# ChazzyGordon/LR2PPO

Hardware: AMD Instinct MI355X
Metric: ppo_steps_per_sec (higher is better)
Workload: dtype f32 (GEMMs: split-bf16 x3 on MFMA, fp32 accumulate); 1 GPU; BASELINE metric 'PPO steps/sec (ViT-B+RoBERTa-base, batch 32)': frames uint8 [32,16,3,224,224] + token ids [32,2,196] -> ViT-B/16 + RoBERTa-base (random weights, inference) -> text_emb [32,2,196,768], img_emb [32,16,768] -> LR2PPO stage-3 rollout + update (actor 519M + critic 526M + reward 526M params); batch_per_gpu=32, tags=2, global_batch=32, parallelism=dp1

## Files before the change

### include/lr2ppo_hip.h

```cpp
#ifndef LR2PPO_HIP_H
#define LR2PPO_HIP_H
#include <stdint.h>

#ifdef __cplusplus
extern "C" {
#endif

#define LR2_ERR_ARG (-1)
#define LR2_ERR_SHAPE (-2)
#define LR2_ERR_LAUNCH (-3)

#define LR2_ABI_VERSION 27
int lr2_abi_version(void);
int lr2_device_info(char* name, int len);

typedef struct lr2_epilogue {
  const void* bias;
  const void* resid;
  const void* aux_z;
  void* out;
  void* out_z;
  void* out_hi;
  uint64_t out_lo_off;
  int32_t ld_planes;
  int32_t ld_resid, ld_aux, ld_out, ld_z;
  int32_t act;
  int32_t accumulate;
  float alpha;
  float drop_p;
  uint32_t drop_site;
  uint32_t _pad;
  uint64_t drop_seed;
  void* adam_p;
  void* adam_m;
  void* adam_v;
  double adam_lr, adam_beta1, adam_beta2, adam_eps, adam_weight_decay;
  void* colsum;
  void* colsum_ws;
  const void* drop_seed_dev;
  const void* adam_lr_dev;
} lr2_epilogue;

int lr2_gemm(const void* A, const void* B, int M, int N, int K, int lda, int ldb, int trans_a, int trans_b,
             uint64_t a_bytes, uint64_t b_bytes, int a_planes, uint64_t a_lo_off, int b_planes, uint64_t b_lo_off,
             const lr2_epilogue* epi, void* splitk_ws, int splits, int block_m, int passes, void* stream);

int lr2_gemm_row_split_plan(int M, int N, int K, int* rows_256, int* tail_block_m);
int lr2_gemm_launch_counts(uint64_t counts[3]);
int lr2_gemm256_tile_rows(int M, int N, int* rows);

int lr2_gather_rows(const void* src, const int64_t* index, void* dst, int B, int t_in, int t_out, uint64_t row_elems,
                    uint64_t src_bstride, uint64_t src_tstride, void* stream);
int lr2_gather_rows_bwd(const void* ddst, const int64_t* index, void* dsrc, int B, int t_in, int t_out,
                        uint64_t row_elems, void* stream);
int lr2_copy_rows(const void* src, void* dst, int dst_planes, uint64_t dst_lo_off, int rows, int D, int group,
                  uint64_t dst_gstride, uint64_t dst_off, void* stream);
int lr2_split_planes(const void* src, void* dst_hi, uint64_t lo_off, uint64_t n, void* stream);
int lr2_split_planes_t(const void* src, void* dst_hi, uint64_t lo_off, int R, int C, void* stream);
int lr2_dropout_planes(const void* src, void* dst_hi, uint64_t lo_off, uint64_t n, float drop_p, uint64_t drop_seed,
                       uint32_t drop_site, void* stream);
typedef struct lr2_split_chunk {
  const void* src;
  void* dst_hi;
  uint64_t lo_off;
  uint64_t count;
} lr2_split_chunk;
int lr2_split_planes_multi(const lr2_split_chunk* table_dev, int n_chunks, void* stream);

int lr2_layernorm_fwd(const void* x, const void* gamma, const void* beta, void* out, void* out_hi, uint64_t out_lo_off,
                      void* mean, void* rstd, int rows, int D, float eps, int mode, int group, uint64_t group_stride,
                      void* stream);

int lr2_layernorm_bwd(const void* dy, int group, uint64_t group_stride, const void* x, const void* gamma, const void* mean,
                      const void* rstd, const void* resid_grad, void* dx, void* dxm_hi, uint64_t dxm_lo_off, float drop_p,
                      uint64_t drop_seed, uint32_t drop_site, const void* drop_seed_dev, void* partials, int nblocks, int rows, int D,
                      int mode, float eps, void* stream);
int lr2_colsum_partials_finish(const void* partials, int nblocks, int cols, int ld, void* out, int accumulate,
                               void* stream);
int lr2_colsum(const void* x, int is_planes, uint64_t lo_off, int rows, int cols, int ld, void* partials, int nblocks,
               void* out, void* stream);

int lr2_xattn_fwd(const void* Q, const void* K, const void* V, void* O, int o_planes, uint64_t o_lo_off, int batch,
                  int heads, int Lq, int Lk, int head_dim, float post_scale, void* stream);
int lr2_xattn_bwd(const void* Q, const void* K, const void* V, const void* dO, void* dQ, void* dK, void* dV,
                  int planes, uint64_t q_lo_off, uint64_t kv_lo_off, int batch, int heads, int Lq, int Lk, int head_dim,
                  float post_scale, void* stream);
int lr2_xattn_fwd_wide(const void* Q, const void* K, const void* V, void* O, int o_planes, uint64_t o_lo_off, int batch,
                       int heads, int Lq, int Lk, int head_dim, float post_scale, void* stream);
int lr2_xattn_bwd_wide(const void* Q, const void* K, const void* V, const void* dO, void* dQ, void* dK, void* dV,
                       int planes, uint64_t q_lo_off, uint64_t kv_lo_off, int batch, int heads, int Lq, int Lk, int head_dim,
                       float post_scale, void* stream);
int lr2_xattn_wide_launch_counts(uint64_t counts[2]);

int lr2_self_attn_fwd(const void* q_hi, const void* k_hi, const void* v_hi, uint64_t lo_off, int ld, const int64_t* seg,
                      void* o, void* o_hi, uint64_t o_lo_off, int ld_o, void* lse, float drop_p, uint64_t drop_seed,
                      uint32_t drop_site, int batch, int heads, int L, int head_dim, float scale, void* stream);

int lr2_first_token_attn(const void* q, int ld_q, const void* k_hi, const void* v_hi, uint64_t lo_off, int ld,
                         const int64_t* seg, void* o, int ld_o, int batch, int heads, int L, int head_dim, float scale,
                         void* stream);

int lr2_self_attn_bwd(const void* q_hi, const void* k_hi, const void* v_hi, uint64_t lo_off, int ld, const void* do_hi,
                      uint64_t do_lo_off, int ld_do, const int64_t* seg, void* dq_hi, void* dk_hi, void* dv_hi,
                      uint64_t d_lo_off, int ld_d, const void* o_hi, uint64_t o_lo_off, int ld_o, void* lse_ws, void* dsum_ws,
                      float drop_p, uint64_t drop_seed, uint32_t drop_site, int batch, int heads, int L, int head_dim, float scale,
                      void* stream);
int lr2_self_attn_plan(int batch, int heads, int L, int ld, int ld_do, int* fwd_persistent, int* bwd_persistent);

int lr2_head_fwd(const void* x, const void* w, const void* b, void* y, int rows, int D, int row_step, int row_off,
                 void* stream);
int lr2_head_bwd(const void* x, const void* w, const void* dy, void* dx, void* dw, void* db, int rows, int D,
                 int row_step, int row_off, int total_rows, void* stream);

int lr2_add_period_rows(const void* x, const void* table, void* out, int rows, int D, int period, void* stream);
int lr2_period_rows_grad(const void* dy, void* dtable, int rows, int D, int period, void* stream);

int lr2_ppo_loss(const void* scores, const void* old_scores, const void* rewards, const void* old_value,
                 const void* value, const int64_t* next_state, int ns_len, int rank_len, int B, int T, float kl_w,
                 float ent_w, float value_clip, float margin, float adv_eps, void* scalars, void* per_item,
                 void* dscores, void* dvalue, void* stats_out, const void* global_stats, int world, void* stream);

int lr2_cls_head_fwd(const void* x, const void* w, const void* b, void* y, int rows, int D, int C, void* stream);
int lr2_cls_head_bwd(const void* x, const void* w, const void* dy, void* dx, void* dw, void* db, int rows, int D, int C,
                     void* stream);
int lr2_cls_scores(const void* logits, void* probs, void* scores, int rows, int C, int use_softmax, void* stream);
int lr2_cls_scores_bwd(const void* probs, const void* scores, const void* dscores, void* dlogits, int rows, int C, void* stream);
int lr2_nll_loss(const void* logits, const int64_t* tgts, int rows, int C, void* loss, void* dlogits, void* stream);

int lr2_smooth_l1(const void* pred, const void* target, int n, float beta, void* loss, void* dpred, void* stream);

int lr2_pair_hinge(const void* scores, int bs, float margin, void* loss_acc, void* dscores, void* stream);

// ... 100 lines not shown
```

### lr2ppo_amd/_native.py

```python
from __future__ import annotations

import ctypes as C
import os
import subprocess
import threading

_HERE = os.path.dirname(os.path.abspath(__file__))
CSRC = os.path.join(_HERE, "csrc")
INCLUDE = os.path.join(os.path.dirname(_HERE), "include")
LIB_PATH = os.path.join(CSRC, "liblr2ppo_hip.so")
SOURCES = ["gemm.hip", "gemm256.hip", "gemm256_mx.hip", "gemm256_b1.hip", "gemm256_f16.hip", "gemm256_tn_b1.hip", "norm.hip", "attn.hip", "attn_wide.hip", "selfattn_fwd.hip", "selfattn_bwd.hip", "first_token_attn.hip", "selfattn_mx.hip", "selfattn_mx_blocked.hip","selfattn_b1_train.hip", "selfattn_b1_blocked.hip", "misc.hip", "fp8.hip", "fp8_train.hip"]
HEADERS = [os.path.join(CSRC, "common.h"), os.path.join(CSRC, "gemm_common.h"), os.path.join(CSRC, "gemm256_ring.h"), os.path.join(CSRC, "fp8_common.h"), os.path.join(CSRC, "selfattn_common.h"), os.path.join(CSRC, "selfattn_b1.h"), os.path.join(INCLUDE, "lr2ppo_hip.h")]
EXTRA_FLAGS = {"attn_wide.hip": ["-fno-slp-vectorize"]}

ABI_VERSION = 27

_lock = threading.Lock()
_lib = None
_lib_override = None


def use_library(path: str):
    global _lib_override
    if _lib is not None:
        raise RuntimeError("lr2ppo_amd: the kernel library is already loaded")
    _lib_override = path


def _stale() -> bool:
    if not os.path.exists(LIB_PATH):
        return True
    t = os.path.getmtime(LIB_PATH)
    deps = [os.path.join(CSRC, s) for s in SOURCES] + HEADERS
    return any(os.path.getmtime(d) > t for d in deps if os.path.exists(d))


def build(force: bool = False, verbose: bool = False) -> str:
    if not force and not _stale():
        return LIB_PATH
    hipcc = os.environ.get("HIPCC", "hipcc")
    objs = []
    procs = []
    for s in SOURCES:
        obj = os.path.join(CSRC, s.replace(".hip", ".o"))
        cmd = [hipcc, "--offload-arch=gfx950", "-O3", "-std=c++17", "-fPIC", *EXTRA_FLAGS.get(s, []), "-I", INCLUDE, "-I", CSRC, "-c",
               os.path.join(CSRC, s), "-o", obj]
        if verbose:
            print(" ".join(cmd))
        procs.append((s, subprocess.Popen(cmd, stdout=subprocess.PIPE, stderr=subprocess.STDOUT)))
        objs.append(obj)
    for s, p in procs:
        out, _ = p.communicate()
        if p.returncode != 0:
            raise RuntimeError(f"hipcc failed on {s}:\n{out.decode(errors='replace')}")
    cmd = [hipcc, "--offload-arch=gfx950", "-shared", "-fPIC", "-o", LIB_PATH] + objs
    r = subprocess.run(cmd, stdout=subprocess.PIPE, stderr=subprocess.STDOUT)
    if r.returncode != 0:
        raise RuntimeError("link failed:\n" + r.stdout.decode(errors="replace"))
    return LIB_PATH


class Epilogue(C.Structure):
    _fields_ = [("bias", C.c_void_p), ("resid", C.c_void_p), ("aux_z", C.c_void_p), ("out", C.c_void_p),
                ("out_z", C.c_void_p), ("out_hi", C.c_void_p), ("out_lo_off", C.c_uint64), ("ld_planes", C.c_int32),
                ("ld_resid", C.c_int32), ("ld_aux", C.c_int32), ("ld_out", C.c_int32),
                ("ld_z", C.c_int32), ("act", C.c_int32), ("accumulate", C.c_int32), ("alpha", C.c_float),
                ("drop_p", C.c_float), ("drop_site", C.c_uint32), ("_pad", C.c_uint32), ("drop_seed", C.c_uint64),
                ("adam_p", C.c_void_p), ("adam_m", C.c_void_p), ("adam_v", C.c_void_p), ("adam_lr", C.c_double),
                ("adam_beta1", C.c_double), ("adam_beta2", C.c_double), ("adam_eps", C.c_double),
                ("adam_weight_decay", C.c_double), ("colsum", C.c_void_p), ("colsum_ws", C.c_void_p), ("drop_seed_dev", C.c_void_p), ("adam_lr_dev", C.c_void_p)]


class SplitChunk(C.Structure):
    _fields_ = [("src", C.c_void_p), ("dst_hi", C.c_void_p), ("lo_off", C.c_uint64), ("count", C.c_uint64)]


class AdamChunk(C.Structure):
    _fields_ = [("p", C.c_void_p), ("g", C.c_void_p), ("m", C.c_void_p), ("v", C.c_void_p), ("count", C.c_uint64),
                ("weight_decay", C.c_float), ("_pad", C.c_float)]


_P, _I, _F, _U64, _U32 = C.c_void_p, C.c_int, C.c_float, C.c_uint64, C.c_uint32

SIGNATURES = {
    "lr2_abi_version": [],
    "lr2_device_info": [C.c_char_p, _I],
    "lr2_gemm": [_P, _P, _I, _I, _I, _I, _I, _I, _I, _U64, _U64, _I, _U64, _I, _U64, C.POINTER(Epilogue), _P, _I, _I, _I, _P],
    "lr2_gemm_row_split_plan": [_I, _I, _I, C.POINTER(C.c_int), C.POINTER(C.c_int)],
    "lr2_gemm_launch_counts": [C.POINTER(C.c_uint64)],
    "lr2_gemm256_tile_rows": [_I, _I, C.POINTER(C.c_int)],
    "lr2_gather_rows": [_P, _P, _P, _I, _I, _I, _U64, _U64, _U64, _P],
    "lr2_gather_rows_bwd": [_P, _P, _P, _I, _I, _I, _U64, _P],
    "lr2_copy_rows": [_P, _P, _I, _U64, _I, _I, _I, _U64, _U64, _P],
    "lr2_split_planes": [_P, _P, _U64, _U64, _P],
    "lr2_dropout_planes": [_P, _P, _U64, _U64, _F, _U64, _U32, _P],
    "lr2_dropout_apply": [_P, _P, _U64, _F, _U64, _U32, _P],
    "lr2_text_embed_bwd": [_P, _P, _P, _P, _P, _P, _P, _P, _I, _I, C.c_int64, _I, _P],
    "lr2_split_planes_t": [_P, _P, _U64, _I, _I, _P],
    "lr2_split_planes_multi": [_P, _I, _P],
    "lr2_layernorm_fwd": [_P, _P, _P, _P, _P, _U64, _P, _P, _I, _I, _F, _I, _I, _U64, _P],
    "lr2_layernorm_bwd": [_P, _I, _U64, _P, _P, _P, _P, _P, _P, _P, _U64, _F, _U64, _U32, _P, _P, _I, _I, _I, _I, _F, _P],
    "lr2_colsum_partials_finish": [_P, _I, _I, _I, _P, _I, _P],
    "lr2_colsum": [_P, _I, _U64, _I, _I, _I, _P, _I, _P, _P],
    "lr2_xattn_fwd": [_P, _P, _P, _P, _I, _U64, _I, _I, _I, _I, _I, _F, _P],
    "lr2_xattn_bwd": [_P, _P, _P, _P, _P, _P, _P, _I, _U64, _U64, _I, _I, _I, _I, _I, _F, _P],
    "lr2_xattn_fwd_wide": [_P, _P, _P, _P, _I, _U64, _I, _I, _I, _I, _I, _F, _P],
    "lr2_xattn_bwd_wide": [_P, _P, _P, _P, _P, _P, _P, _I, _U64, _U64, _I, _I, _I, _I, _I, _F, _P],
    "lr2_xattn_wide_launch_counts": [C.POINTER(C.c_uint64)],
    "lr2_self_attn_fwd": [_P, _P, _P, _U64, _I, _P, _P, _P, _U64, _I, _P, _F, _U64, _U32, _I, _I, _I, _I, _F, _P],
    "lr2_first_token_attn": [_P, _I, _P, _P, _U64, _I, _P, _P, _I, _I, _I, _I, _I, _F, _P],
    "lr2_self_attn_bwd": [_P, _P, _P, _U64, _I, _P, _U64, _I, _P, _P, _P, _P, _U64, _I, _P, _U64, _I, _P, _P, _F, _U64, _U32, _I,
                          _I, _I, _I, _F, _P],
    "lr2_self_attn_plan": [_I, _I, _I, _I, _I, C.POINTER(C.c_int), C.POINTER(C.c_int)],
    "lr2_head_fwd": [_P, _P, _P, _P, _I, _I, _I, _I, _P],
    "lr2_head_bwd": [_P, _P, _P, _P, _P, _P, _I, _I, _I, _I, _I, _P],
    "lr2_add_period_rows": [_P, _P, _P, _I, _I, _I, _P],
    "lr2_period_rows_grad": [_P, _P, _I, _I, _I, _P],
    "lr2_ppo_loss": [_P, _P, _P, _P, _P, _P, _I, _I, _I, _I, _F, _F, _F, _F, _F, _P, _P, _P, _P, _P, _P, _I, _P],
    "lr2_smooth_l1": [_P, _P, _I, _F, _P, _P, _P],
    "lr2_cls_head_fwd": [_P, _P, _P, _P, _I, _I, _I, _P],
    "lr2_cls_head_bwd": [_P, _P, _P, _P, _P, _P, _I, _I, _I, _P],
    "lr2_cls_scores": [_P, _P, _P, _I, _I, _I, _P],
    "lr2_cls_scores_bwd": [_P, _P, _P, _P, _I, _I, _P],
    "lr2_nll_loss": [_P, _P, _I, _I, _P, _P, _P],
    "lr2_pair_hinge": [_P, _I, _F, _P, _P, _P],
    "lr2_adamw_multi": [_P, _I, C.c_double, C.c_double, C.c_double, C.c_double, _P, _P],
    "lr2_step_scalars_store": [_P, _U64, _P, _I, _P],
    "lr2_quant_mxfp8": [_P, _I, _P, _P, _I, _I, _P],
    "lr2_layernorm_fwd_mxfp8": [_P, _P, _P, _P, _P, _P, _I, _I, _F, _I, _P],
    "lr2_gemm_mxfp8": [_P, _P, _P, _P, _P, _I, _P, _P, _I, _I, _P, _P, _P, _U64, _I, _I, _I, _I, _P],
    "lr2_quant_mxfp8_t": [_P, _I, _U64, _I, _P, _I, _I, _P, _P, _P, _P, _P, _P, _I, _I, _I, _P],
    "lr2_gemm_mxfp8_wgrad": [_P, _P, _P, _P, _P, _I, _I, _P, _I, _I, _I, _I, _P],
    "lr2_dropout_residual": [_P, _P, _P, _U64, _F, _U64, _U32, _P],
    "lr2_self_attn_fwd_bf16": [_P, _P, _P, _I, _P, _P, _P, _P, _P, _I, _I, _I, _I, _I, _F, _P],
    "lr2_self_attn_fwd_bf16_plan": [_I, _I, _I, _I, C.POINTER(C.c_int)],
    "lr2_gemm_bf16": [_P, _P, _I, _I, _I, _I, _I, _U64, _U64, C.POINTER(Epilogue), _I, _P],
    "lr2_gemm_bf16_launch_counts": [C.POINTER(C.c_uint64)],
    "lr2_gemm_bf16_train": [_P, _P, _I, _I, _I, _I, _I, _I, _I, _U64, _U64, C.POINTER(Epilogue), _P, _I, _I, _P],
    "lr2_gemm_bf16_train_launch_counts": [C.POINTER(C.c_uint64)],
    "lr2_self_attn_fwd_bf16_train": [_P, _P, _P, _I, _P, _P, _I, _P, _F, _U64, _U32, _I, _I, _I, _I, _F, _P],
    "lr2_self_attn_bwd_bf16": [_P, _P, _P, _I, _P, _I, _P, _P, _P, _P, _I, _P, _P, _F, _U64, _U32, _I, _I, _I, _I, _F, _P],
    "lr2_self_attn_bf16_train_launch_counts": [C.POINTER(C.c_uint64)],
    "lr2_self_attn_fwd_bf16_train_blocked": [_P, _P, _P, _I, _P, _P, _I, _P, _F, _U64, _U32, _I, _I, _I, _I, _F, _P],
    "lr2_self_attn_bwd_bf16_blocked": [_P, _P, _P, _I, _P, _I, _P, _P, _P, _P, _I, _P, _P, _F, _U64, _U32, _I, _I, _I, _I, _F, _P],
    "lr2_self_attn_bf16_blocked_plan": [_I, C.POINTER(C.c_int), C.POINTER(C.c_int), C.POINTER(C.c_int)],
    "lr2_self_attn_bf16_blocked_launch_counts": [C.POINTER(C.c_uint64)],
    "lr2_self_attn_fwd_bf16_blocked": [_P, _P, _P, _I, _P, _P, _P, _P, _P, _I, _I, _I, _I, _I, _F, _P],
    "lr2_self_attn_fwd_bf16_blocked_launch_count": [C.POINTER(C.c_uint64)],
    "lr2_gemm_f16": [_P, _P, _I, _I, _I, _I, _I, _U64, _U64, C.POINTER(Epilogue), _P],
    "lr2_gemm_f16_launch_count": [C.POINTER(C.c_uint64)],
    "lr2_gemm_f16_tiled": [_P, _P, _I, _I, _I, _I, _I, _U64, _U64, C.POINTER(Epilogue), _I, _P],
    "lr2_gemm_f16_launch_counts": [C.POINTER(C.c_uint64)],
    "lr2_layernorm_fwd_f16": [_P, _P, _P, _P, _P, _P, _P, _I, _I, _F, _I, _I, _U64, _P],
    "lr2_round_f16": [_P, _P, _U64, _P],
    "lr2_self_attn_fwd_f16": [_P, _P, _P, _I, _P, _P, _P, _I, _I, _I, _I, _I, _F, _P],
    "lr2_self_attn_fwd_f16_launch_count": [C.POINTER(C.c_uint64)],
    "lr2_self_attn_fwd_f16_blocked": [_P, _P, _P, _I, _P, _P, _P, _I, _I, _I, _I, _I, _F, _P],
    "lr2_self_attn_fwd_f16_blocked_launch_count": [C.POINTER(C.c_uint64)],
    "lr2_text_embed": [_P, _P, _P, _P, _P, _P, _I, _I, _I, C.c_int64, _I, _P, _P],
    "lr2_patchify_planes": [_P, _I, _P, _U64, _I, _I, _I, _I, _I, _I, C.POINTER(C.c_float), C.POINTER(C.c_float), _P],
    "lr2_ndcg": [_P, _P, _P, _P, _P, _I, _P, _I, _P],
    "lr2_patchify": [_P, _P, _I, _I, _I, _I, _I, _P],
    "lr2_vit_assemble": [_P, _P, _P, _P, _I, _I, _I, _P],
}


def lib() -> C.CDLL:
    global _lib
    if _lib is not None:
        return _lib
    with _lock:
        if _lib is not None:
            return _lib
# ... 37 lines not shown
```

### lr2ppo_amd/csrc/gemm256.hip

```cpp
#include "gemm256_ring.h"

namespace lr2gemm {
namespace g256 {

using namespace ring256;
constexpr int BM = 256, BN = 256, BK = 32;
constexpr int LDS_BYTES = RING;

struct SplitProducts {
  template <int AH, int BH, int MIH>
  static __device__ __forceinline__ void mfma_section(f32x4_t (&acc)[2 * MIH][4], const bf16x8_t (&ahi)[MIH], const bf16x8_t (&alo)[MIH],
                                                      const bf16x8_t (&bhi)[2], const bf16x8_t (&blo)[2]) {
    __builtin_amdgcn_s_setprio(1);
#pragma unroll
    for (int j = 0; j < 2; ++j)
#pragma unroll
      for (int i = 0; i < MIH; ++i)
        acc[AH * MIH + i][BH * 2 + j] = __builtin_amdgcn_mfma_f32_16x16x32_bf16(alo[i], bhi[j], acc[AH * MIH + i][BH * 2 + j], 0, 0, 0);
#pragma unroll
    for (int j = 0; j < 2; ++j)
#pragma unroll
      for (int i = 0; i < MIH; ++i)
        acc[AH * MIH + i][BH * 2 + j] = __builtin_amdgcn_mfma_f32_16x16x32_bf16(ahi[i], blo[j], acc[AH * MIH + i][BH * 2 + j], 0, 0, 0);
#pragma unroll
    for (int j = 0; j < 2; ++j)
#pragma unroll
      for (int i = 0; i < MIH; ++i)
        acc[AH * MIH + i][BH * 2 + j] = __builtin_amdgcn_mfma_f32_16x16x32_bf16(ahi[i], bhi[j], acc[AH * MIH + i][BH * 2 + j], 0, 0, 0);
    __builtin_amdgcn_s_setprio(0);
    section_barrier();
  }
};

template <int MIH>
__global__ __launch_bounds__(512, 2) void gemm256_nt_kernel(GemmParams g) {
  constexpr int BMT = 64 * MIH, WMT = 32 * MIH;
  extern __shared__ __attribute__((aligned(16))) char smem[];
  const int tid = threadIdx.x;
  const int lane = tid & 63;
  const int wave = __builtin_amdgcn_readfirstlane(tid >> 6);
  const int wr = wave >> 2, wc = wave & 3;

  int tm, tn;
  tile_coords(g.tiles_m, g.tiles_n, blockIdx.x, tm, tn);
  const int m0 = tm * BMT, n0 = tn * BN;

  Ctx<TwoPlanes> c;
  c.nt = g.K / BK;
  c.src.a = uniform_rsrc(g.A, g.a_bytes);
  c.src.a2 = uniform_rsrc((const char*)g.A + g.a_lo_off, g.a_bytes);
  c.src.b = uniform_rsrc(g.B, g.b_bytes);
  c.src.b2 = uniform_rsrc((const char*)g.B + g.b_lo_off, g.b_bytes);
  lane_setup<MIH>(c, smem, m0, n0, wave, lane, (uint64_t)g.lda * 2u, (uint64_t)g.ldb * 2u, g.M, g.N);

  f32x4_t acc[2 * MIH][4];
#pragma unroll
  for (int i = 0; i < 2 * MIH; ++i)
#pragma unroll
    for (int j = 0; j < 4; ++j) acc[i][j] = f32x4_t{0.f, 0.f, 0.f, 0.f};

  prologue<NoExtras>(c, wr);
  for (int t = 0; t < c.nt; t += 2) {
    k_step_bf16<SplitProducts, 0, MIH>(c, t, acc);
    if (t + 1 < c.nt) k_step_bf16<SplitProducts, 1, MIH>(c, t + 1, acc);
  }
  drain(wr);

  float* slab = reinterpret_cast<float*>(smem) + wave * (32 * (64 + 4));
  epilogue_wave<WMT, 64, 2 * MIH, 4, 1>(g, acc, slab, m0 + wr * WMT, n0 + wc * 64, lane, nullptr);
}

}

namespace g256t {

using g256::BK;
using g256::BM;
using g256::BN;
using ring256::OOB;
constexpr int PLANE = 32 * 256;
constexpr int STAGE_STRIDE = 2 * PLANE;
constexpr int HALF_STRIDE = 2 * STAGE_STRIDE;
constexpr int REGION = 2 * HALF_STRIDE;
constexpr int LDS_BYTES = 2 * REGION;

__device__ __forceinline__ int swz_tr16(int k) { return ((((k & 3) | (((k >> 3) & 1) << 2))) << 1) & 15; }

template <int IMM>
__device__ __forceinline__ bf16x8_t lds_read_tr(uint32_t addr) {
  u32x2_t lo, hi;
  asm volatile("ds_read_b64_tr_b16 %0, %1 offset:%2" : "=v"(lo) : "v"(addr), "i"(IMM));
  asm volatile("ds_read_b64_tr_b16 %0, %1 offset:%2" : "=v"(hi) : "v"(addr), "i"(IMM + 4 * 256));
  u32x4_t v = {lo[0], lo[1], hi[0], hi[1]};
  return __builtin_bit_cast(bf16x8_t, v);
}

struct Ctx {
  __amdgpu_buffer_rsrc_t a_hi, a_lo, b_hi, b_lo;
  uint32_t voff_a[2], voff_b[2];
  uint32_t kstep_a, kstep_b;
  uint32_t rd_a[4], rd_b[2];
  char* smem;
  int wave, nt;
};

template <bool IS_A, int HALF>
__device__ __forceinline__ void issue_part(const Ctx& c, int tile, int stage) {
  const uint32_t base = IS_A ? c.voff_a[HALF] : c.voff_b[HALF];
  const uint32_t step = IS_A ? c.kstep_a : c.kstep_b;
  const uint64_t o = (uint64_t)base + (uint64_t)(uint32_t)tile * (uint64_t)step;
  const uint32_t v = (tile < c.nt && base != OOB && o < (uint64_t)OOB) ? (uint32_t)o : OOB;
  char* dst = c.smem + (IS_A ? 0 : REGION) + HALF * HALF_STRIDE + stage * STAGE_STRIDE + c.wave * 1024;
  __builtin_amdgcn_raw_ptr_buffer_load_lds(IS_A ? c.a_hi : c.b_hi, LDS_PTR(dst), 16, v, 0, 0, 0);
  __builtin_amdgcn_raw_ptr_buffer_load_lds(IS_A ? c.a_lo : c.b_lo, LDS_PTR(dst + PLANE), 16, v, 0, 0, 0);
}

template <int HALF, int S>
__device__ __forceinline__ void read_a_half(const Ctx& c, bf16x8_t (&hi)[4], bf16x8_t (&lo)[4]) {
  constexpr int O = HALF * HALF_STRIDE + S * STAGE_STRIDE;
  hi[0] = lds_read_tr<O>(c.rd_a[0]);
  hi[1] = lds_read_tr<O>(c.rd_a[1]);
  hi[2] = lds_read_tr<O>(c.rd_a[2]);
  hi[3] = lds_read_tr<O>(c.rd_a[3]);
  lo[0] = lds_read_tr<O + PLANE>(c.rd_a[0]);
  lo[1] = lds_read_tr<O + PLANE>(c.rd_a[1]);
  lo[2] = lds_read_tr<O + PLANE>(c.rd_a[2]);
  lo[3] = lds_read_tr<O + PLANE>(c.rd_a[3]);
}
template <int HALF, int S>
__device__ __forceinline__ void read_b_half(const Ctx& c, bf16x8_t (&hi)[2], bf16x8_t (&lo)[2]) {
  constexpr int O = HALF * HALF_STRIDE + S * STAGE_STRIDE;
  hi[0] = lds_read_tr<O>(c.rd_b[0]);
  hi[1] = lds_read_tr<O>(c.rd_b[1]);
  lo[0] = lds_read_tr<O + PLANE>(c.rd_b[0]);
  lo[1] = lds_read_tr<O + PLANE>(c.rd_b[1]);
}

__device__ __forceinline__ float frag_sum(const bf16x8_t& f) {
  const u32x4_t w = __builtin_bit_cast(u32x4_t, f);
  float s = 0.f;
#pragma unroll
  for (int d = 0; d < 4; ++d) s += __uint_as_float(w[d] << 16) + __uint_as_float(w[d] & 0xffff0000u);
  return s;
}
template <int AH>
__device__ __forceinline__ void colsum_frags(float (&cs)[2], int wc, const bf16x8_t (&ahi)[4], const bf16x8_t (&alo)[4]) {
  if (wc == 0) cs[AH] += frag_sum(ahi[0]) + frag_sum(alo[0]);
  else if (wc == 1) cs[AH] += frag_sum(ahi[1]) + frag_sum(alo[1]);
  else if (wc == 2) cs[AH] += frag_sum(ahi[2]) + frag_sum(alo[2]);
  else cs[AH] += frag_sum(ahi[3]) + frag_sum(alo[3]);
}

// ... 65 lines not shown
    const int sx = swz_tr16(ka);
    const uint32_t sm = (uint32_t)(uintptr_t)(__attribute__((address_space(3))) char*)smem;
    const uint32_t rowb = (uint32_t)(ka * 256 + 8 * (pp & 1));
#pragma unroll
    for (int i = 0; i < 4; ++i) c.rd_a[i] = sm + rowb + (uint32_t)((((wr * 8 + 2 * i + (pp >> 1)) ^ sx)) * 16);
#pragma unroll
    for (int j = 0; j < 2; ++j) c.rd_b[j] = sm + REGION + rowb + (uint32_t)((((wc * 4 + 2 * j + (pp >> 1)) ^ sx)) * 16);
  }

  f32x4_t acc[8][4];
#pragma unroll
  for (int i = 0; i < 8; ++i)
#pragma unroll
    for (int j = 0; j < 4; ++j) acc[i][j] = f32x4_t{0.f, 0.f, 0.f, 0.f};

  issue_part<true, 0>(c, 0, 0);
  issue_part<false, 1>(c, 0, 0);
  issue_part<true, 1>(c, 0, 0);
  issue_part<false, 0>(c, 0, 0);
  issue_part<true, 0>(c, 1, 1);
  issue_part<false, 1>(c, 1, 1);
  issue_part<true, 1>(c, 1, 1);
  ring256::end_load_section<6>();
  if (wr == 1) {
    __builtin_amdgcn_s_barrier();
    __builtin_amdgcn_sched_barrier(0);
  }
  float cs[2] = {0.f, 0.f};
  const bool cs_on = g.epi.colsum_partial != nullptr;
  int cs_phase = (t0 + g.tiles_n - tn) % g.tiles_n;
  for (int t = 0; t < c.nt; t += 2) {
    k_step<0>(c, t, acc, cs, wc, cs_on && cs_phase == 0);
    cs_phase = cs_phase + 1 == g.tiles_n ? 0 : cs_phase + 1;
    if (t + 1 < c.nt) k_step<1>(c, t + 1, acc, cs, wc, cs_on && cs_phase == 0);
    cs_phase = cs_phase + 1 == g.tiles_n ? 0 : cs_phase + 1;
  }
  if (wr == 0) {
    __builtin_amdgcn_s_barrier();
    __builtin_amdgcn_sched_barrier(0);
  }
  asm volatile("s_waitcnt vmcnt(0)" ::: "memory");
  __builtin_amdgcn_s_barrier();
  __builtin_amdgcn_sched_barrier(0);

  if (cs_on) {
    float* dst = g.epi.colsum_partial + (size_t)(split * g.tiles_n + tn) * (size_t)g.M;
#pragma unroll
    for (int h = 0; h < 2; ++h) {
      float v = cs[h];
      v += __shfl_xor(v, 16, 64);
      v += __shfl_xor(v, 32, 64);
      const int m = m0 + wr * 128 + h * 64 + wc * 16 + (lane & 15);
      if (lane < 16 && m < g.M) dst[m] = v;
    }
  }
  float* slab = reinterpret_cast<float*>(smem) + wave * (32 * (64 + 4));
  float* partial = g.partial ? g.partial + (size_t)split * (size_t)g.M * (size_t)g.N : nullptr;
  epilogue_wave<128, 64, 8, 4, 1>(g, acc, slab, m0 + wr * 128, n0 + wc * 64, lane, partial);
}

}

int launch_gemm256_tn(const GemmParams& p_in, int splits, hipStream_t stream) {
  using namespace g256t;
  GemmParams p = p_in;
  p.tiles_m = (p.M + BM - 1) / BM;
  p.tiles_n = (p.N + BN - 1) / BN;
  p.splits = splits;
  static bool attr_set = false;
  if (!attr_set) {
    if (lr2_allow_dynamic_lds(gemm256_tn_kernel, LDS_BYTES, "gemm256_tn")) return LR2_ERR_LAUNCH;
    attr_set = true;
  }
  LR2_LAUNCH(gemm256_tn_kernel, dim3(p.tiles_m * p.tiles_n * splits), dim3(512), LDS_BYTES, stream, p);
  return lr2_launch_status(__func__);
}

int gemm256_nt_tile_rows(int M, int N) {
  const int tn = (N + g256::BN - 1) / g256::BN;
  const int t256 = ((M + 255) / 256) * tn, t192 = ((M + 191) / 192) * tn;
  return (t256 < 256 && t192 <= 256 && t192 > t256) ? 192 : 256;
}

int launch_gemm256_nt(const GemmParams& p_in, hipStream_t stream) {
  using namespace g256;
  GemmParams p = p_in;
  const int bm = gemm256_nt_tile_rows(p.M, p.N);
  p.tiles_m = (p.M + bm - 1) / bm;
  p.tiles_n = (p.N + BN - 1) / BN;
  static bool attr_set = false;
  if (!attr_set) {
    if (lr2_allow_dynamic_lds(gemm256_nt_kernel<4>, LDS_BYTES, "gemm256")) return LR2_ERR_LAUNCH;
    if (lr2_allow_dynamic_lds(gemm256_nt_kernel<3>, LDS_BYTES, "gemm256(192 rows)")) return LR2_ERR_LAUNCH;
    attr_set = true;
  }
  if (bm == 192) LR2_LAUNCH(gemm256_nt_kernel<3>, dim3(p.tiles_m * p.tiles_n), dim3(512), LDS_BYTES, stream, p);
  else LR2_LAUNCH(gemm256_nt_kernel<4>, dim3(p.tiles_m * p.tiles_n), dim3(512), LDS_BYTES, stream, p);
  return lr2_launch_status(__func__);
}

}
```

### lr2ppo_amd/csrc/gemm256_ring.h

```cpp
#pragma once
#include "gemm_common.h"

namespace lr2gemm {
namespace ring256 {

constexpr int PLANE = 128 * 64;
constexpr int PART = 2 * PLANE;
constexpr int STAGE = 4 * PART;
constexpr int RING = 2 * STAGE;
constexpr int SLOT_A0 = 0, SLOT_B0 = 1, SLOT_B1 = 2, SLOT_A1 = 3;
constexpr uint32_t OOB = 0xFFFFFF00u;

__device__ __forceinline__ int swz(int r) { return (4 - ((r >> 2) & 3)) & 3; }

template <int IMM>
__device__ __forceinline__ u32x4_t lds_read16(uint32_t addr) {
  u32x4_t v;
  asm volatile("ds_read_b128 %0, %1 offset:%2" : "=v"(v) : "v"(addr), "i"(IMM));
  return v;
}

__device__ __forceinline__ void section_barrier() {
  __builtin_amdgcn_sched_barrier(0);
  __builtin_amdgcn_s_barrier();
// ... 69 lines not shown
  const uint32_t v0 = in ? base + (uint32_t)tile * SRC::STEP : OOB;
  const uint32_t v1 = in ? v0 + SRC::SECOND : OOB;
  char* dst = c.smem + stage * STAGE + SLOT * PART + c.wave * 1024;
  dma16(IS_A ? c.src.a : c.src.b, dst, v0);
  dma16(c.src.template second<IS_A>(), dst + PLANE, v1);
}

template <int SLOT, int MIH, class V>
__device__ __forceinline__ void read_a_half(uint32_t base, V (&p0)[MIH], V (&p1)[MIH]) {
  p0[0] = __builtin_bit_cast(V, lds_read16<SLOT * PART + 0 * 1024>(base));
  p0[1] = __builtin_bit_cast(V, lds_read16<SLOT * PART + 1 * 1024>(base));
  p0[2] = __builtin_bit_cast(V, lds_read16<SLOT * PART + 2 * 1024>(base));
  if constexpr (MIH == 4) p0[3] = __builtin_bit_cast(V, lds_read16<SLOT * PART + 3 * 1024>(base));
  p1[0] = __builtin_bit_cast(V, lds_read16<SLOT * PART + PLANE + 0 * 1024>(base));
  p1[1] = __builtin_bit_cast(V, lds_read16<SLOT * PART + PLANE + 1 * 1024>(base));
  p1[2] = __builtin_bit_cast(V, lds_read16<SLOT * PART + PLANE + 2 * 1024>(base));
  if constexpr (MIH == 4) p1[3] = __builtin_bit_cast(V, lds_read16<SLOT * PART + PLANE + 3 * 1024>(base));
}
template <int SLOT, class V>
__device__ __forceinline__ void read_b_half(uint32_t base, V (&p0)[2], V (&p1)[2]) {
  p0[0] = __builtin_bit_cast(V, lds_read16<SLOT * PART + 0 * 1024>(base));
  p0[1] = __builtin_bit_cast(V, lds_read16<SLOT * PART + 1 * 1024>(base));
  p1[0] = __builtin_bit_cast(V, lds_read16<SLOT * PART + PLANE + 0 * 1024>(base));
  p1[1] = __builtin_bit_cast(V, lds_read16<SLOT * PART + PLANE + 1 * 1024>(base));
}

template <class PRODUCTS, int S, int MIH, class CTX>
__device__ __forceinline__ void k_step_bf16(const CTX& c, int t, f32x4_t (&acc)[2 * MIH][4]) {
  bf16x8_t a0[MIH], a1[MIH], b0[2], b1[2];
  issue_part<SLOT_B0, false, 0>(c, t + 1, S ^ 1);
  read_a_half<SLOT_A0, MIH>(c.rd_a[S], a0, a1);
  read_b_half<SLOT_B0>(c.rd_b[S], b0, b1);
  end_load_section<12>();
  PRODUCTS::template mfma_section<0, 0, MIH>(acc, a0, a1, b0, b1);
  issue_part<SLOT_A0, true, 0>(c, t + 2, S);
  read_b_half<SLOT_B1>(c.rd_b[S], b0, b1);
  end_load_section<12>();
  PRODUCTS::template mfma_section<0, 1, MIH>(acc, a0, a1, b0, b1);
  issue_part<SLOT_B1, false, 1>(c, t + 2, S);
  read_a_half<SLOT_A1, MIH>(c.rd_a[S], a0, a1);
  end_load_section<12>();
  PRODUCTS::template mfma_section<1, 1, MIH>(acc, a0, a1, b0, b1);
  issue_part<SLOT_A1, true, 1>(c, t + 2, S);
  read_b_half<SLOT_B0>(c.rd_b[S], b0, b1);
  end_load_section<6>();
  PRODUCTS::template mfma_section<1, 0, MIH>(acc, a0, a1, b0, b1);
}

struct NoExtras {
  static constexpr int FIRST_WAIT = 6;
  template <class CTX> static __device__ __forceinline__ void begin(const CTX&) {}
  template <class CTX> static __device__ __forceinline__ void after_a1(const CTX&, int) {}
};

template <class EXTRAS, class CTX>
__device__ __forceinline__ void prologue(const CTX& c, int wr) {
  EXTRAS::begin(c);
  issue_part<SLOT_A0, true, 0>(c, 0, 0);
  issue_part<SLOT_B1, false, 1>(c, 0, 0);
  issue_part<SLOT_A1, true, 1>(c, 0, 0);
  EXTRAS::after_a1(c, 0);
  issue_part<SLOT_B0, false, 0>(c, 0, 0);
  issue_part<SLOT_A0, true, 0>(c, 1, 1);
  issue_part<SLOT_B1, false, 1>(c, 1, 1);
  issue_part<SLOT_A1, true, 1>(c, 1, 1);
  EXTRAS::after_a1(c, 1);
  end_load_section<EXTRAS::FIRST_WAIT>();
  if (wr == 1) {
    __builtin_amdgcn_s_barrier();
    __builtin_amdgcn_sched_barrier(0);
  }
}

__device__ __forceinline__ void drain(int wr) {
  if (wr == 0) {
    __builtin_amdgcn_s_barrier();
    __builtin_amdgcn_sched_barrier(0);
  }
  asm volatile("s_waitcnt vmcnt(0)" ::: "memory");
  __builtin_amdgcn_s_barrier();
  __builtin_amdgcn_sched_barrier(0);
}

}
}
```

### lr2ppo_amd/ops.py

```python
from __future__ import annotations

import contextlib
import ctypes as C
import functools
import os
from typing import Optional

import torch

from . import _native as _nat

_PASSES = 3


def set_gemm_passes(p: int):
    global _PASSES
    if p not in (1, 3):
        raise ValueError("passes must be 1 or 3")
    _PASSES = p


def get_gemm_passes() -> int:
    return _PASSES

# ... 395 lines not shown
    e.bias, e.resid, e.out = _ptr(bias), _ptr(resid), _ptr(out)
    e.ld_resid, e.ld_out = _ld(resid, N), (N if ld_out is None else ld_out)
    if out_plane is not None:
        e.out_hi, e.out_lo_off, e.ld_planes = _plane_ptr(out_plane, M * N, "gemm_bf16: out_plane"), 0, N
    elif out_planes is not None:
        if out_planes.rows != M or planes_col < 0 or planes_col % 4 or planes_col + N > out_planes.cols:
            raise ValueError("gemm_bf16: out_planes must be [M, >= planes_col + N], planes_col a multiple of 4")
        e.out_hi, e.out_lo_off, e.ld_planes = out_planes.data_ptr() + 2 * planes_col, out_planes.lo_off, out_planes.cols
    e.act, e.alpha = act, alpha
    if block_m is None:
        block_m = 256 if use_gemm256_b1(M, N, K) else _bf16_fallback_block_m(M, N)
    with _Timed(f"gemm_bf16_M{M}_N{N}_K{K}", 2.0 * M * N * K, 2.0 * (M * K + N * K) + (4.0 if out is not None else 2.0) * M * N):
        rc = _nat.lib().lr2_gemm_bf16(a_ptr, b_ptr, M, N, K, lda, ldb, a.numel() * 2, b.numel() * 2, C.byref(e), block_m, _stream())
    if rc:
        _nat.check(rc, f"lr2_gemm_bf16(M={M},N={N},K={K},block_m={block_m})")
    return out if out is not None else (out_plane if out_plane is not None else out_planes)


def gemm_bf16_launch_counts():
    c = (C.c_uint64 * 2)()
    _nat.check(_nat.lib().lr2_gemm_bf16_launch_counts(c), "lr2_gemm_bf16_launch_counts")
    return int(c[0]), int(c[1])


def gemm_f16(a: torch.Tensor, b: torch.Tensor, out: Optional[torch.Tensor], M: int, N: int, K: int, *,
             lda: Optional[int] = None, ldb: Optional[int] = None, ld_out: Optional[int] = None, bias: Optional[torch.Tensor] = None,
             act: int = 0, resid: Optional[torch.Tensor] = None, alpha: float = 1.0, out_plane: Optional[torch.Tensor] = None,
             out_planes: Optional[Planes] = None, planes_col: int = 0, block_m: Optional[int] = None):
    _chk_f32(out, bias, resid)
    lda = K if lda is None else lda
    ldb = K if ldb is None else ldb
    a_ptr = _plane_ptr(a, (M - 1) * lda + K, "gemm_f16: a")
    b_ptr = _plane_ptr(b, (N - 1) * ldb + K, "gemm_f16: b")
    if out_plane is not None and out_planes is not None:
        raise ValueError("gemm_f16: out_plane excludes out_planes")
    e = _nat.Epilogue()
    e.bias, e.resid, e.out = _ptr(bias), _ptr(resid), _ptr(out)
    e.ld_resid, e.ld_out = _ld(resid, N), (N if ld_out is None else ld_out)
    if out_plane is not None:
        e.out_hi, e.out_lo_off, e.ld_planes = _plane_ptr(out_plane, M * N, "gemm_f16: out_plane"), 0, N
    elif out_planes is not None:
        if out_planes.rows != M or planes_col < 0 or planes_col % 4 or planes_col + N > out_planes.cols:
            raise ValueError("gemm_f16: out_planes must be [M, >= planes_col + N], planes_col a multiple of 4")
        e.out_hi, e.out_lo_off, e.ld_planes = out_planes.data_ptr() + 2 * planes_col, out_planes.lo_off, out_planes.cols
    e.act, e.alpha = act, alpha
    with _Timed(f"gemm_f16_M{M}_N{N}_K{K}", 2.0 * M * N * K, 2.0 * (M * K + N * K) + (4.0 if out is not None else 2.0) * M * N):
        if block_m is None:
            rc = _nat.lib().lr2_gemm_f16(a_ptr, b_ptr, M, N, K, lda, ldb, a.numel() * 2, b.numel() * 2, C.byref(e), _stream())
        else:
            if block_m not in (256, 128, 64):
                raise ValueError("gemm_f16: block_m is None, 256, 128 or 64")
            rc = _nat.lib().lr2_gemm_f16_tiled(a_ptr, b_ptr, M, N, K, lda, ldb, a.numel() * 2, b.numel() * 2, C.byref(e), block_m,
                                               _stream())
    if rc:
        _nat.check(rc, f"lr2_gemm_f16(M={M},N={N},K={K},block_m={block_m})")
    return out if out is not None else (out_plane if out_plane is not None else out_planes)


def gemm_f16_launch_count() -> int:
    c = C.c_uint64(0)
    _nat.check(_nat.lib().lr2_gemm_f16_launch_count(C.byref(c)), "lr2_gemm_f16_launch_count")
    return int(c.value)


def gemm_f16_launch_counts():
    c = (C.c_uint64 * 2)()
    _nat.check(_nat.lib().lr2_gemm_f16_launch_counts(c), "lr2_gemm_f16_launch_counts")
    return int(c[0]), int(c[1])


_F16_FORCE_256 = False


@contextlib.contextmanager
def f16_force_256():
    global _F16_FORCE_256
    prev, _F16_FORCE_256 = _F16_FORCE_256, True
    try:
        yield
    finally:
        _F16_FORCE_256 = prev


def f16_schedule_block_m(M: int, N: int, K: int) -> Optional[int]:
    return None if _F16_FORCE_256 else f16_block_m(M, N, K)


@functools.lru_cache(maxsize=4096)
def f16_block_m(M: int, N: int, K: int) -> int:
    if K % 64:
        return 64
    tiles = ((M + 255) // 256) * ((N + 255) // 256)
    return 256 if tiles >= 128 else 64


def layernorm_fwd_f16(x, gamma, beta, rows, D, eps, mode, *, group=0, group_stride=0, out=None, mean=None, rstd=None,
                      out_plane: Optional[torch.Tensor] = None):
    _chk_f32(x, gamma, beta, out, mean, rstd)
    if out is None and out_plane is None:
        raise ValueError("layernorm_fwd_f16: out and / or out_plane")
    hp = _plane_ptr(out_plane, rows * D, "layernorm_fwd_f16: out_plane") if out_plane is not None else None
    with _Timed(f"lnfwd_f16_R{rows}_D{D}", 0.0, (6.0 if out is None else 10.0 if out_plane is not None else 8.0) * rows * D):
        rc = _nat.lib().lr2_layernorm_fwd_f16(x.data_ptr(), gamma.data_ptr(), beta.data_ptr(), _ptr(out), hp, _ptr(mean), _ptr(rstd),
                                              rows, D, eps, mode, group, group_stride, _stream())
    _nat.check(rc, "lr2_layernorm_fwd_f16")
    return out if out is not None else out_plane


def round_f16(src: torch.Tensor, dst: torch.Tensor) -> torch.Tensor:
    _chk_f32(src)
    n = src.numel()
    with _Timed(f"round_f16_{n}", 0.0, 6.0 * n):
        rc = _nat.lib().lr2_round_f16(src.data_ptr(), _plane_ptr(dst, n, "round_f16: dst"), n, _stream())
    _nat.check(rc, "lr2_round_f16")
    return dst


def self_attn_fwd_f16(qkv: torch.Tensor, seg, *, batch, heads, L, head_dim, scale, out: Optional[torch.Tensor] = None,
                      out_plane: Optional[torch.Tensor] = None):
    E = heads * head_dim
    if qkv.element_size() != 2 or not qkv.is_cuda or qkv.numel() < batch * L * 3 * E:
        raise TypeError("self_attn_fwd_f16: qkv is a 2-byte HIP tensor [batch * L, 3 * heads * head_dim]")
    if seg.dtype != torch.int64:
        raise TypeError("seg must be int64")
    _chk_f32(out)
    if out is None and out_plane is None:
        raise ValueError("self_attn_fwd_f16: out and / or out_plane")
    ob = _plane_ptr(out_plane, batch * L * E, "self_attn_fwd_f16: out_plane") if out_plane is not None else None
    base = qkv.data_ptr()
    with _Timed(f"selfattn_f16_B{batch}_H{heads}_L{L}", 4.0 * batch * heads * L * L * head_dim, 7.0 * batch * L * E):
        _nat.check(_nat.lib().lr2_self_attn_fwd_f16(base, base + 2 * E, base + 4 * E, 3 * E, seg.data_ptr(), _ptr(out), ob, E, batch,
                                                    heads, L, head_dim, scale, _stream()), "lr2_self_attn_fwd_f16")
    return out if out is not None else out_plane


def self_attn_fwd_f16_launch_count() -> int:
    c = C.c_uint64(0)
    _nat.check(_nat.lib().lr2_self_attn_fwd_f16_launch_count(C.byref(c)), "lr2_self_attn_fwd_f16_launch_count")
    return int(c.value)


def self_attn_fwd_f16_blocked(qkv: torch.Tensor, seg, *, batch, heads, L, head_dim, scale, out: Optional[torch.Tensor] = None,
                              out_plane: Optional[torch.Tensor] = None):
    E = heads * head_dim
    if qkv.element_size() != 2 or not qkv.is_cuda or qkv.numel() < batch * L * 3 * E:
        raise TypeError("self_attn_fwd_f16_blocked: qkv is a 2-byte HIP tensor [batch * L, 3 * heads * head_dim]")
    if seg.dtype != torch.int64:
        raise TypeError("seg must be int64")
    _chk_f32(out)
    if out is None and out_plane is None:
        raise ValueError("self_attn_fwd_f16_blocked: out and / or out_plane")
    ob = _plane_ptr(out_plane, batch * L * E, "self_attn_fwd_f16_blocked: out_plane") if out_plane is not None else None
    base = qkv.data_ptr()
    with _Timed(f"selfattn_f16l_B{batch}_H{heads}_L{L}", 4.0 * batch * heads * L * L * head_dim, 7.0 * batch * L * E):
        _nat.check(_nat.lib().lr2_self_attn_fwd_f16_blocked(base, base + 2 * E, base + 4 * E, 3 * E, seg.data_ptr(), _ptr(out), ob, E,
                                                            batch, heads, L, head_dim, scale, _stream()), "lr2_self_attn_fwd_f16_blocked")
    return out if out is not None else out_plane


def self_attn_fwd_f16_blocked_launch_count() -> int:
    c = C.c_uint64(0)
    _nat.check(_nat.lib().lr2_self_attn_fwd_f16_blocked_launch_count(C.byref(c)), "lr2_self_attn_fwd_f16_blocked_launch_count")
    return int(c.value)


_BF16_TRAIN_FORCE_256 = False
# ... 706 lines not shown
```

Baseline: 14.36 PPO steps/s (1 step = ViT-B/16 over 32 x 16 frames + RoBERTa-base over 32 x 2 tag sequences, frozen, in line -> 1 rollout batch + 1 update minibatch, 32 items x 2 tags per GPU; head_only_steps_per_sec = the same step on pre-extracted features).

## Add persistent 256x256 NT GEMM kernel that prefetches next tile during tail

Adds a persistent variant of the 256-row NT GEMM kernel that launches one workgroup per CU and walks multiple output tiles. The last K-steps of each tile issue loads for the next tile's first stages, so the next tile's prologue overlaps the current epilogue and launch/ramp costs are amortised. By default it is used only for large GEMMs (at least 4x CU-count tiles) whose epilogue loads nothing extra (no residual, accumulate or Adam). It reserves extra LDS for the epilogue slab, which may lower occupancy, and the cross-tile pipeline adds synchronisation complexity.

Result: no change. 14.45 PPO steps/s (1 step = ViT-B/16 over 32 x 16 frames + RoBERTa-base over 32 x 2 tag sequences, frozen, in line -> 1 rollout batch + 1 update minibatch, 32 items x 2 tags per GPU; head_only_steps_per_sec = the same step on pre-extracted features) (median of 6 runs) (+0.6%).

```diff
diff --git a/include/lr2ppo_hip.h b/include/lr2ppo_hip.h
--- a/include/lr2ppo_hip.h
+++ b/include/lr2ppo_hip.h
@@ -48,6 +48,8 @@
 int lr2_gemm_row_split_plan(int M, int N, int K, int* rows_256, int* tail_block_m);
 int lr2_gemm_launch_counts(uint64_t counts[3]);
 int lr2_gemm256_tile_rows(int M, int N, int* rows);
+int lr2_gemm256_persist_plan(int M, int N, int K);
+int lr2_gemm256_persist(int mode, int workgroups);
 
 int lr2_gather_rows(const void* src, const int64_t* index, void* dst, int B, int t_in, int t_out, uint64_t row_elems,
                     uint64_t src_bstride, uint64_t src_tstride, void* stream);
diff --git a/lr2ppo_amd/_native.py b/lr2ppo_amd/_native.py
--- a/lr2ppo_amd/_native.py
+++ b/lr2ppo_amd/_native.py
@@ -89,6 +89,8 @@
     "lr2_gemm_row_split_plan": [_I, _I, _I, C.POINTER(C.c_int), C.POINTER(C.c_int)],
     "lr2_gemm_launch_counts": [C.POINTER(C.c_uint64)],
     "lr2_gemm256_tile_rows": [_I, _I, C.POINTER(C.c_int)],
+    "lr2_gemm256_persist_plan": [_I, _I, _I],
+    "lr2_gemm256_persist": [_I, _I],
     "lr2_gather_rows": [_P, _P, _P, _I, _I, _I, _U64, _U64, _U64, _P],
     "lr2_gather_rows_bwd": [_P, _P, _P, _I, _I, _I, _U64, _P],
     "lr2_copy_rows": [_P, _P, _I, _U64, _I, _I, _I, _U64, _U64, _P],
diff --git a/lr2ppo_amd/csrc/gemm256.hip b/lr2ppo_amd/csrc/gemm256.hip
--- a/lr2ppo_amd/csrc/gemm256.hip
+++ b/lr2ppo_amd/csrc/gemm256.hip
@@ -68,6 +68,85 @@
 
   float* slab = reinterpret_cast<float*>(smem) + wave * (32 * (64 + 4));
   epilogue_wave<WMT, 64, 2 * MIH, 4, 1>(g, acc, slab, m0 + wr * WMT, n0 + wc * 64, lane, nullptr);
+}
+
+template <int FORM>
+__global__ __launch_bounds__(512, 2) void gemm256_nt_persist_kernel(GemmParams g) {
+  constexpr int MIH = 4, BMT = 64 * MIH, WMT = 32 * MIH;
+  extern __shared__ __attribute__((aligned(16))) char smem[];
+  const int total = g.tiles_m * g.tiles_n;
+  int v = blockIdx.x;
+  if (v >= total) return;
+  const int tid = threadIdx.x;
+  const int lane = tid & 63;
+  const int wave = __builtin_amdgcn_readfirstlane(tid >> 6);
+  const int wr = wave >> 2, wc = wave & 3;
+  const uint64_t pitch_a = (uint64_t)g.lda * 2u, pitch_b = (uint64_t)g.ldb * 2u;
+
+  int tm, tn;
+  tile_coords(g.tiles_m, g.tiles_n, v, tm, tn);
+  int m0 = tm * BMT, n0 = tn * BN;
+
+  Ctx<TwoPlanes> c;
+  c.nt = g.K / BK;
+  c.src.a = uniform_rsrc(g.A, g.a_bytes);
+  c.src.a2 = uniform_rsrc((const char*)g.A + g.a_lo_off, g.a_bytes);
+  c.src.b = uniform_rsrc(g.B, g.b_bytes);
+  c.src.b2 = uniform_rsrc((const char*)g.B + g.b_lo_off, g.b_bytes);
+  lane_setup<MIH>(c, smem, m0, n0, wave, lane, pitch_a, pitch_b, g.M, g.N);
+  float* slab = reinterpret_cast<float*>(smem + WALK_KEEP) + wave * (32 * (64 + 4));
+
+  for (bool first = true;; first = false) {
+    const int vn = v + (int)gridDim.x;
+    const bool more = vn < total;
+    int m0n = 0, n0n = 0;
+    if (more) {
+      tile_coords(g.tiles_m, g.tiles_n, vn, tm, tn);
+      m0n = tm * BMT;
+      n0n = tn * BN;
+    }
+    NextTile nx;
+    next_tile_offsets<MIH>(c, nx, more, m0n, n0n, lane, pitch_a, pitch_b, g.M, g.N);
+
+    f32x4_t acc[2 * MIH][4];
+#pragma unroll
+    for (int i = 0; i < 2 * MIH; ++i)
+#pragma unroll
+      for (int j = 0; j < 4; ++j) acc[i][j] = f32x4_t{0.f, 0.f, 0.f, 0.f};
+
+    if (first) prologue<NoExtras>(c, wr);
+    else walk_skew(wr);
+    for (int t = 0; t < c.nt - 2; t += 2) {
+      k_step_bf16_stage0<SplitProducts, MIH>(c, t, acc, !first && t == 0);
+      k_step_bf16<SplitProducts, 1, MIH>(c, t + 1, acc);
+    }
+    k_step_walk<SplitProducts, 0, MIH>(c, nx, acc, !first && c.nt == 2);
+    k_step_walk<SplitProducts, 1, MIH>(c, nx, acc, false);
+    drain(wr);
+
+    GemmParams ge = g;
+    if constexpr (FORM >= 1) {
+      ge.epi.aux_z = nullptr;
+      ge.epi.accumulate = 0;
+      ge.epi.adam_p = nullptr;
+    }
+    if constexpr (FORM == 1) {
+      ge.epi.resid = nullptr;
+      ge.epi.act = g.epi.act & 1u;
+    }
+    epilogue_wave<WMT, 64, 2 * MIH, 4, 1>(ge, acc, slab, m0 + wr * WMT, n0 + wc * 64, lane, nullptr);
+    if (!more) break;
+    walk_release();
+#pragma unroll
+    for (int h = 0; h < 2; ++h) {
+      c.voff_a[h] = nx.voff_a[h];
+      c.voff_b[h] = nx.voff_b[h];
+    }
+    walk_restart(c);
+    m0 = m0n;
+    n0 = n0n;
+    v = vn;
+  }
 }
 
 }
@@ -299,21 +378,71 @@
   return (t256 < 256 && t192 <= 256 && t192 > t256) ? 192 : 256;
 }
 
+static int persist_cus() {
+  static int cached[64] = {0};
+  int dev = 0;
+  if (hipGetDevice(&dev) != hipSuccess || dev < 0 || dev >= 64) {
+    (void)hipGetLastError();
+    return 256;
+  }
+  if (cached[dev] == 0) {
+    int n = 0;
+    if (hipDeviceGetAttribute(&n, hipDeviceAttributeMultiprocessorCount, dev) != hipSuccess || n < 8) n = 256;
+    (void)hipGetLastError();
+    cached[dev] = n & ~7;
+  }
+  return cached[dev];
+}
+
+static int g_persist_mode = 1;
+static int g_persist_wg = 0;
+
+int gemm256_persist_workgroups(int M, int N, int K) {
+  if (g_persist_mode == 0 || M <= 0 || N <= 0 || K <= 0 || (K % 64) != 0) return 0;
+  const int G = g_persist_wg > 0 ? g_persist_wg : persist_cus();
+  if (g_persist_mode == 2) return G;
+  const long long tiles = (long long)((M + 255) / 256) * (long long)((N + g256::BN - 1) / g256::BN);
+  return (gemm256_nt_tile_rows(M, N) == 256 && tiles >= 4ll * G) ? G : 0;
+}
+
+static int persist_form(const GemmParams& p) {
+  const Epilogue& e = p.epi;
+  const bool loads = e.act == 2 || e.resid || e.accumulate;
+  return (!loads && !e.adam_p) ? 1 : 0;
+}
+
 int launch_gemm256_nt(const GemmParams& p_in, hipStream_t stream) {
   using namespace g256;
   GemmParams p = p_in;
-  const int bm = gemm256_nt_tile_rows(p.M, p.N);
+  int wg = gemm256_persist_workgroups(p.M, p.N, p.K);
+  if (g_persist_mode == 1 && persist_form(p) == 0) wg = 0;
+  const int bm = wg > 0 ? 256 : gemm256_nt_tile_rows(p.M, p.N);
   p.tiles_m = (p.M + bm - 1) / bm;
   p.tiles_n = (p.N + BN - 1) / BN;
   static bool attr_set = false;
   if (!attr_set) {
     if (lr2_allow_dynamic_lds(gemm256_nt_kernel<4>, LDS_BYTES, "gemm256")) return LR2_ERR_LAUNCH;
     if (lr2_allow_dynamic_lds(gemm256_nt_kernel<3>, LDS_BYTES, "gemm256(192 rows)")) return LR2_ERR_LAUNCH;
+    if (lr2_allow_dynamic_lds(gemm256_nt_persist_kernel<0>, ring256::WALK_LDS, "gemm256(persistent)")) return LR2_ERR_LAUNCH;
+    if (lr2_allow_dynamic_lds(gemm256_nt_persist_kernel<1>, ring256::WALK_LDS, "gemm256(persistent, no loads)")) return LR2_ERR_LAUNCH;
+    (void)persist_cus();
     attr_set = true;
   }
-  if (bm == 192) LR2_LAUNCH(gemm256_nt_kernel<3>, dim3(p.tiles_m * p.tiles_n), dim3(512), LDS_BYTES, stream, p);
+  if (wg > 0) {
+    if (persist_form(p) == 1) LR2_LAUNCH(gemm256_nt_persist_kernel<1>, dim3(wg), dim3(512), ring256::WALK_LDS, stream, p);
+    else LR2_LAUNCH(gemm256_nt_persist_kernel<0>, dim3(wg), dim3(512), ring256::WALK_LDS, stream, p);
+  } else if (bm == 192) LR2_LAUNCH(gemm256_nt_kernel<3>, dim3(p.tiles_m * p.tiles_n), dim3(512), LDS_BYTES, stream, p);
   else LR2_LAUNCH(gemm256_nt_kernel<4>, dim3(p.tiles_m * p.tiles_n), dim3(512), LDS_BYTES, stream, p);
   return lr2_launch_status(__func__);
 }
 
 }
+
+extern "C" int lr2_gemm256_persist_plan(int M, int N, int K) { return lr2gemm::gemm256_persist_workgroups(M, N, K); }
+
+extern "C" int lr2_gemm256_persist(int mode, int workgroups) {
+  if (mode < 0 || mode > 2 || workgroups < 0 || workgroups > 65535) return LR2_ERR_ARG;
+  lr2gemm::g_persist_mode = mode;
+  lr2gemm::g_persist_wg = workgroups;
+  return 0;
+}
diff --git a/lr2ppo_amd/csrc/gemm256_ring.h b/lr2ppo_amd/csrc/gemm256_ring.h
--- a/lr2ppo_amd/csrc/gemm256_ring.h
+++ b/lr2ppo_amd/csrc/gemm256_ring.h
@@ -175,5 +175,102 @@
   __builtin_amdgcn_sched_barrier(0);
 }
 
-}
-}
+constexpr int WALK_KEEP = STAGE + PART;
+constexpr int WALK_SLAB = 32 * (64 + 4) * 4;
+constexpr int WALK_LDS = WALK_KEEP + 8 * WALK_SLAB;
+
+struct NextTile {
+  uint32_t voff_a[2], voff_b[2];
+};
+template <int MIH, class CTX>
+__device__ __forceinline__ void next_tile_offsets(const CTX& c, NextTile& nx, bool more, int m0, int n0, int lane, uint64_t pitch_a,
+                                                  uint64_t pitch_b, int M, int N) {
+  CTX t = c;
+  lane_setup<MIH>(t, c.smem, m0, n0, c.wave, lane, pitch_a, pitch_b, M, N);
+#pragma unroll
+  for (int h = 0; h < 2; ++h) {
+    nx.voff_a[h] = more ? t.voff_a[h] : OOB;
+    nx.voff_b[h] = more ? t.voff_b[h] : OOB;
+  }
+}
+
+template <int SLOT, bool IS_A, class CTX>
+__device__ __forceinline__ void issue_part_from(const CTX& c, uint32_t base, int k, int stage) {
+  using SRC = typename CTX::Src;
+  const bool in = base != OOB;
+  const uint32_t v0 = in ? base + (uint32_t)k * SRC::STEP : OOB;
+  const uint32_t v1 = in ? v0 + SRC::SECOND : OOB;
+  char* dst = c.smem + stage * STAGE + SLOT * PART + c.wave * 1024;
+  dma16(IS_A ? c.src.a : c.src.b, dst, v0);
+  dma16(c.src.template second<IS_A>(), dst + PLANE, v1);
+}
+
+__device__ __forceinline__ void end_load_section_landed(bool landed) {
+  if (!landed) __builtin_amdgcn_s_waitcnt(12 | (7 << 4) | (15 << 8));
+  end_load_section<63>();
+}
+template <class PRODUCTS, int MIH, class CTX>
+__device__ __forceinline__ void k_step_bf16_stage0(const CTX& c, int t, f32x4_t (&acc)[2 * MIH][4], bool landed) {
+  bf16x8_t a0[MIH], a1[MIH], b0[2], b1[2];
+  issue_part<SLOT_B0, false, 0>(c, t + 1, 1);
+  read_a_half<SLOT_A0, MIH>(c.rd_a[0], a0, a1);
+  read_b_half<SLOT_B0>(c.rd_b[0], b0, b1);
+  end_load_section_landed(landed);
+  PRODUCTS::template mfma_section<0, 0, MIH>(acc, a0, a1, b0, b1);
+  issue_part<SLOT_A0, true, 0>(c, t + 2, 0);
+  read_b_half<SLOT_B1>(c.rd_b[0], b0, b1);
+  end_load_section_landed(landed);
+  PRODUCTS::template mfma_section<0, 1, MIH>(acc, a0, a1, b0, b1);
+  issue_part<SLOT_B1, false, 1>(c, t + 2, 0);
+  read_a_half<SLOT_A1, MIH>(c.rd_a[0], a0, a1);
+  end_load_section_landed(landed);
+  PRODUCTS::template mfma_section<1, 1, MIH>(acc, a0, a1, b0, b1);
+  issue_part<SLOT_A1, true, 1>(c, t + 2, 0);
+  read_b_half<SLOT_B0>(c.rd_b[0], b0, b1);
+  end_load_section<6>();
+  PRODUCTS::template mfma_section<1, 0, MIH>(acc, a0, a1, b0, b1);
+}
+
+template <class PRODUCTS, int LAST, int MIH, class CTX>
+__device__ __forceinline__ void k_step_walk(const CTX& c, const NextTile& nx, f32x4_t (&acc)[2 * MIH][4], bool landed) {
+  constexpr int S = LAST;
+  bf16x8_t a0[MIH], a1[MIH], b0[2], b1[2];
+  if constexpr (LAST == 0) issue_part<SLOT_B0, false, 0>(c, c.nt - 1, 1);
+  else issue_part_from<SLOT_B0, false>(c, nx.voff_b[0], 0, 0);
+  read_a_half<SLOT_A0, MIH>(c.rd_a[S], a0, a1);
+  read_b_half<SLOT_B0>(c.rd_b[S], b0, b1);
+  end_load_section_landed(LAST == 0 && landed);
+  PRODUCTS::template mfma_section<0, 0, MIH>(acc, a0, a1, b0, b1);
+  issue_part_from<SLOT_A0, true>(c, nx.voff_a[0], LAST, S);
+  read_b_half<SLOT_B1>(c.rd_b[S], b0, b1);
+  end_load_section_landed(LAST == 0 && landed);
+  PRODUCTS::template mfma_section<0, 1, MIH>(acc, a0, a1, b0, b1);
+  issue_part_from<SLOT_B1, false>(c, LAST == 0 ? nx.voff_b[1] : OOB, 0, S);
+  read_a_half<SLOT_A1, MIH>(c.rd_a[S], a0, a1);
+  end_load_section_landed(LAST == 0 && landed);
+  PRODUCTS::template mfma_section<1, 1, MIH>(acc, a0, a1, b0, b1);
+  issue_part_from<SLOT_A1, true>(c, LAST == 0 ? nx.voff_a[1] : OOB, 0, S);
+  read_b_half<SLOT_B0>(c.rd_b[S], b0, b1);
+  end_load_section<6>();
+  PRODUCTS::template mfma_section<1, 0, MIH>(acc, a0, a1, b0, b1);
+}
+
+__device__ __forceinline__ void walk_release() {
+  asm volatile("s_waitcnt lgkmcnt(0)" ::: "memory");
+  section_barrier();
+}
+template <class CTX>
+__device__ __forceinline__ void walk_restart(const CTX& c) {
+  issue_part<SLOT_B1, false, 1>(c, 1, 1);
+  issue_part<SLOT_A1, true, 1>(c, 1, 1);
+}
+__device__ __forceinline__ void walk_skew(int wr) {
+  __builtin_amdgcn_sched_barrier(0);
+  if (wr == 1) {
+    __builtin_amdgcn_s_barrier();
+    __builtin_amdgcn_sched_barrier(0);
+  }
+}
+
+}
+}
diff --git a/lr2ppo_amd/ops.py b/lr2ppo_amd/ops.py
--- a/lr2ppo_amd/ops.py
+++ b/lr2ppo_amd/ops.py
@@ -501,6 +501,26 @@
         _F16_FORCE_256 = prev
 
 
+_GEMM256_PERSIST = (1, 0)
+
+
+@contextlib.contextmanager
+def gemm256_persist(mode: int, workgroups: int = 0):
+    global _GEMM256_PERSIST
+    prev = _GEMM256_PERSIST
+    _nat.check(_nat.lib().lr2_gemm256_persist(mode, workgroups), f"lr2_gemm256_persist({mode}, {workgroups})")
+    _GEMM256_PERSIST = (mode, workgroups)
+    try:
+        yield
+    finally:
+        _nat.check(_nat.lib().lr2_gemm256_persist(*prev), "lr2_gemm256_persist")
+        _GEMM256_PERSIST = prev
+
+
+def gemm256_persist_plan(M: int, N: int, K: int) -> int:
+    return int(_nat.lib().lr2_gemm256_persist_plan(M, N, K))
+
+
 def f16_schedule_block_m(M: int, N: int, K: int) -> Optional[int]:
     return None if _F16_FORCE_256 else f16_block_m(M, N, K)
 
```
